# lzzcd001/MeshDiffusion

Hardware: NVIDIA H100
Metric: denoising sample-steps/sec at res-64 (4x64^3), uncond_gen PC sampler (higher is better)
Workload: dtype bf16x3

## Files before the change

### meshdiffusion_b200/csrc/gemm_tc.cuh

```cuda
#pragma once
#include "ptx.cuh"
#include "act_format.cuh"
#include "gn_stats.cuh"

namespace mdb {

constexpr int kBlockM = 128;
constexpr int kRowBytes = 128;
constexpr int kAStageRows = 160;
constexpr int kAStageBytes = kAStageRows * kRowBytes;
constexpr int kMaxLoads = 2048;
constexpr int kMaxAMaps = 16;
constexpr int kGemmThreads = 384;
constexpr int kEpiThreads = 256;

struct __align__(16) LoadEntry {
  uint8_t tmap;
  uint8_t nk;
  uint8_t rows;
  uint8_t jrows;
  int8_t dx, dy, dz;
  uint8_t wsrc;
  uint16_t c0;
  uint16_t wc0;
  uint8_t tap0;
  uint8_t tapj;
  uint8_t tmap_lo;
  uint8_t pad;
};
static_assert(sizeof(LoadEntry) == 16, "LoadEntry must be 16 bytes");

struct GemmSeg {
  int n_groups;
  int nk;
  int a_bytes;
  int a_stride;
  int jbytes;
};
constexpr int kMaxSegs = 8;

struct GemmParams {
  CUtensorMap amap[kMaxAMaps];
  CUtensorMap bmap;
  const LoadEntry* loads;
  int n_loads;
  int n_segs;
  GemmSeg segs[kMaxSegs];
  int bx, by, bz, bb;
  int X, Y, Z, Bn;
  int tx, ty, tz, tb;
  int n_tiles_n;
  int N;
  int b_batched;
  int splits;
  int total_groups;
  float* partial;
  long long split_stride;
  int batch_fastest;
  int kb_elems;
  int b_explicit_k;
  int b_kstep;
  int b_lo_k;
  int n_aslots, a_slot_bytes, n_bslots, b_slot_bytes;
  long long out_lo_off, res_lo_off;
  void* out;
  long long osx, osy, osz, osb;
  long long ocs;
  int out_fp32;
  int round_out;
  const float* bias;
  int bias_on_m;
  const float* rowbias;
  long long rowbias_ld;
  const void* res;
  long long rsx, rsy, rsz, rsb;
  int res_fp32;
  float alpha;
  long long* stats;
  const void* res1;
  long long r1sx, r1sy, r1sz, r1sb;
  long long res1_lo_off;
  int res_c0;
  const float4* gnb_c;
  int gnb_silu;
  int gnb_drop_thresh; float gnb_drop_scale; unsigned long long gnb_seed;
  float* gnb_part;
};

constexpr int kMaxSlots = 8;
constexpr int kMaxDynSmem = 232448;
template <int BLOCK_N, bool kWholeTile = false>
struct GemmCfg {
  static constexpr int kBTileBytes = BLOCK_N * kRowBytes;
  static constexpr int kStatsFloats = 24 * BLOCK_N;
  static constexpr int kStageCols = (kWholeTile || BLOCK_N < 64) ? BLOCK_N : 64;
  static constexpr int kStageRounds = BLOCK_N / kStageCols;
  static_assert(kStageRounds <= 2, "the epilogue stages at most two rounds");
  static constexpr int kAccPitch = kStageCols + 4;
  static constexpr int kAccFloats = kBlockM * kAccPitch;
  static constexpr int kFixedBytes = 1024 + kAccFloats * 4 + kStatsFloats * 4 + 4 * kMaxSlots * 8;
};
constexpr int kRegsProducer = 40, kRegsConsumer = 232;

__device__ __forceinline__ uint64_t kdesc(uint32_t saddr) { return make_wgmma_desc(saddr, 16, 1024); }

template <int OFF>
__device__ __forceinline__ void colsum_butterfly(float (&s)[32], float (&ss)[32], int lane) {
  const bool hi = (lane & OFF) != 0;
#pragma unroll
  for (int i = 0; i < OFF; ++i) {
    const float send_s = hi ? s[i] : s[i + OFF];
    const float send_q = hi ? ss[i] : ss[i + OFF];
    const float keep_s = hi ? s[i + OFF] : s[i];
    const float keep_q = hi ? ss[i + OFF] : ss[i];
    s[i] = keep_s + __shfl_xor_sync(0xffffffffu, send_s, OFF);
    ss[i] = keep_q + __shfl_xor_sync(0xffffffffu, send_q, OFF);
  }
  if constexpr (OFF > 1) colsum_butterfly<OFF / 2>(s, ss, lane);
}

template <int BLOCK_N, bool TF32, bool GNB = false, bool X3 = false>
__global__ void __launch_bounds__(kGemmThreads, 1) gemm_tc_kernel(const __grid_constant__ GemmParams p) {
  using Cfg = GemmCfg<BLOCK_N, GNB>;
  constexpr int kParts = X3 ? 2 : 1;
  const int NA = p.n_aslots, NB = p.n_bslots;
  const uint32_t a_slot = (uint32_t)p.a_slot_bytes, b_slot = (uint32_t)p.b_slot_bytes;
  extern __shared__ uint8_t smem_raw[];
  uint8_t* smem = reinterpret_cast<uint8_t*>((reinterpret_cast<uintptr_t>(smem_raw) + 1023) & ~uintptr_t(1023));
  float* s_acc = reinterpret_cast<float*>(smem + NA * p.a_slot_bytes + NB * p.b_slot_bytes);
  float* s_stats = s_acc + Cfg::kAccFloats;
  uint64_t* bars = reinterpret_cast<uint64_t*>(s_stats + Cfg::kStatsFloats);

  const uint32_t a_ring = smem_u32(smem), b_ring = a_ring + NA * a_slot;
  const uint32_t a_full = smem_u32(bars), a_empty = a_full + 8 * kMaxSlots;
  const uint32_t b_full = a_empty + 8 * kMaxSlots, b_empty = b_full + 8 * kMaxSlots;

  const int warp = __shfl_sync(0xffffffffu, (int)(threadIdx.x >> 5), 0), lane = threadIdx.x & 31;

  if (warp == 0 && lane == 0) {
    for (int i = 0; i < kMaxAMaps; ++i) tma_prefetch_desc(&p.amap[i]);
    tma_prefetch_desc(&p.bmap);
  }
  if (warp == 1 && lane == 0) {
    for (int i = 0; i < NA; ++i) { mbar_init(a_full + 8 * i, 1); mbar_init(a_empty + 8 * i, 2); }
    for (int i = 0; i < NB; ++i) { mbar_init(b_full + 8 * i, 1); mbar_init(b_empty + 8 * i, 2); }
    fence_barrier_init();
    fence_proxy_async();
  }
  __syncthreads();

  const int tiles_m = p.tx * p.ty * p.tz * p.tb;
  const int splits = p.splits > 1 ? p.splits : 1;
  const int total_tiles = tiles_m * p.n_tiles_n * splits;
  const int first_tile = (int)blockIdx.x;
  const int tile_step = (int)gridDim.x;

  auto split_range = [&](int item, int& lo, int& hi) {
    const int sidx = item % splits;
    lo = (int)((long long)p.total_groups * sidx / splits);
    hi = (int)((long long)p.total_groups * (sidx + 1) / splits);
  };
  int mt_of_tile = 0;
  auto decode = [&](int tile, int& x0, int& y0, int& z0, int& b0, int& n0) {
    tile /= splits;
    int nt = tile % p.n_tiles_n;
    int mt = tile / p.n_tiles_n;
    mt_of_tile = mt;
    n0 = nt * BLOCK_N;
    int bt = 0;
    if (p.batch_fastest) { bt = mt % p.tb; mt /= p.tb; }
    int xt = mt % p.tx; mt /= p.tx;
    int yt = mt % p.ty; mt /= p.ty;
    int zt = mt % p.tz; mt /= p.tz;
    if (!p.batch_fastest) bt = mt;
    x0 = xt * p.bx; y0 = yt * p.by; z0 = zt * p.bz; b0 = bt * p.bb;
  };

  if (warp < 4) {
    setmaxnreg_dec<kRegsProducer>();
    if (warp == 0) {
      uint32_t as = 0, aph = 0, bs = 0, bph = 0;
      for (int tile = first_tile; tile < total_tiles; tile += tile_step) {
        int x0, y0, z0, b0, n0;
        decode(tile, x0, y0, z0, b0, n0);
        int kcol = 0, l = 0, gi = 0, g_lo, g_hi;
        split_range(tile, g_lo, g_hi);
        const int bcoord = p.b_batched ? b0 : 0;
        for (int sg = 0; sg < p.n_segs; ++sg) {
          const GemmSeg& seg = p.segs[sg];
          for (int g = 0; g < seg.n_groups; ++g, ++gi) {
            if (gi < g_lo || gi >= g_hi) {
              kcol += seg.nk * p.b_kstep;
              ++l;
              continue;
            }
            const uint4 raw = __ldg(reinterpret_cast<const uint4*>(p.loads + l));
            const LoadEntry& en = reinterpret_cast<const LoadEntry&>(raw);
            mbar_wait(a_empty + 8 * as, aph ^ 1);
            if (elect_one()) {
              const uint32_t abase = a_ring + as * a_slot, bar = a_full + 8 * as;
              mbar_expect_tx(bar, kParts * seg.a_bytes);
              tma_load_5d(&p.amap[en.tmap], bar, abase, en.c0, x0 + en.dx, y0 + en.dy, z0 + en.dz, b0);
              if constexpr (X3) tma_load_5d(&p.amap[en.tmap_lo], bar, abase + seg.a_stride, en.c0, x0 + en.dx, y0 + en.dy, z0 + en.dz, b0);
            }
            __syncwarp();
            if (++as == (uint32_t)NA) { as = 0; aph ^= 1; }
            int kc = (X3 && p.b_explicit_k) ? (int)en.wc0 : kcol;
            for (int j = 0; j < seg.nk; ++j) {
              mbar_wait(b_empty + 8 * bs, bph ^ 1);
              if (elect_one()) {
                const uint32_t bbase = b_ring + bs * b_slot, bar = b_full + 8 * bs;
                mbar_expect_tx(bar, kParts * Cfg::kBTileBytes);
                tma_load_3d(&p.bmap, bar, bbase, kc, n0, bcoord);
                if constexpr (X3) tma_load_3d(&p.bmap, bar, bbase + Cfg::kBTileBytes, kc + p.b_lo_k, n0, bcoord);
              }
              __syncwarp();
              kc += p.b_kstep;
              if (++bs == (uint32_t)NB) { bs = 0; bph ^= 1; }
            }
            kcol += seg.nk * p.b_kstep;
            ++l;
          }
        }
      }
    }
  } else {
    setmaxnreg_inc<kRegsConsumer>();
    const int wg = (warp - 4) >> 2;
    const int wt = threadIdx.x & 127;
    const int q = warp & 3;
    const int half = (warp - 4) >> 2;
    constexpr int kChunks = BLOCK_N / 32;
    constexpr int kChunkStep = kChunks >= 2 ? 2 : 1;
    const int row = q * 32 + lane;
    const int et = threadIdx.x - 128;
    const int rows_per_b = p.bx * p.by * p.bz;
    const int seg = row / rows_per_b;
    int it = 0;
    int staged_n0 = -1, staged_b0 = -1, bias_buf = 0;
    int want_cols = 0;
    if constexpr (GNB) {
      want_cols = (p.stats != nullptr || p.gnb_part != nullptr) ? 1 : 0;
      asm volatile("" : "+r"(want_cols));
    }
    uint32_t as = 0, aph = 0, bs = 0, bph = 0;
    for (int tile = first_tile; tile < total_tiles; tile += tile_step, ++it) {
      const int vit = it;
      constexpr int kAccRegs = X3 ? BLOCK_N : BLOCK_N / 2;
      float acc[kAccRegs];
      float (&acc_hi)[BLOCK_N / 2] = *reinterpret_cast<float (*)[BLOCK_N / 2]>(acc);
#pragma unroll
      for (int i = 0; i < kAccRegs; ++i) acc[i] = 0.f;
      {
        int gi = 0, g_lo, g_hi;
        split_range(tile, g_lo, g_hi);
        int prev_b = -1, prev_a = -1;
        const uint32_t a_row0 = (uint32_t)wg * 64 * kRowBytes;
        for (int sg = 0; sg < p.n_segs; ++sg) {
          const GemmSeg& sgm = p.segs[sg];
          for (int g = 0; g < sgm.n_groups; ++g, ++gi) {
            if (gi < g_lo || gi >= g_hi) continue;
            mbar_wait(a_full + 8 * as, aph);
            const uint32_t abase = a_ring + as * a_slot + a_row0;
            for (int j = 0; j < sgm.nk; ++j) {
              mbar_wait(b_full + 8 * bs, bph);
              const uint64_t ad = kdesc(abase + j * sgm.jbytes);
              const uint64_t bd = kdesc(b_ring + bs * b_slot);
              wgmma_fence();
              if constexpr (X3) {
                const uint64_t adl = kdesc(abase + sgm.a_stride + j * sgm.jbytes);
#pragma unroll
                for (int k = 0; k < kRowBytes / 32; ++k) wgmma_kmajor<2 * BLOCK_N, false>(acc, ad + 2 * k, bd + 2 * k, 1u);
                wgmma_fence();
#pragma unroll
                for (int k = 0; k < kRowBytes / 32; ++k) wgmma_kmajor<BLOCK_N, false>(acc_hi, adl + 2 * k, bd + 2 * k, 1u);
              } else {
#pragma unroll
                for (int k = 0; k < kRowBytes / 32; ++k) wgmma_kmajor<BLOCK_N, TF32>(acc, ad + 2 * k, bd + 2 * k, 1u);
              }
              wgmma_commit();
              wgmma_wait<1>();
              if (wt == 0) {
                if (prev_b >= 0) mbar_arrive(b_empty + 8 * prev_b);
                if (prev_a >= 0) mbar_arrive(a_empty + 8 * prev_a);
              }
              prev_b = (int)bs;
              prev_a = j + 1 == sgm.nk ? (int)as : -1;
              if (++bs == (uint32_t)NB) { bs = 0; bph ^= 1; }
            }
            if (++as == (uint32_t)NA) { as = 0; aph ^= 1; }
          }
        }
        wgmma_wait<0>();
        fence_operands(acc);
        if (wt == 0) {
          if (prev_b >= 0) mbar_arrive(b_empty + 8 * prev_b);
          if (prev_a >= 0) mbar_arrive(a_empty + 8 * prev_a);
        }
        if constexpr (X3) {
#pragma unroll
          for (int i = 0; i < BLOCK_N / 2; ++i) acc[i] += acc[BLOCK_N / 2 + i];
        }
      }
      int x0, y0, z0, b0, n0;
      decode(tile, x0, y0, z0, b0, n0);
      int r = row;
      const int xl = r % p.bx; r /= p.bx;
      const int yl = r % p.by; r /= p.by;
      const int zl = r % p.bz; r /= p.bz;
      const int xg = x0 + xl, yg = y0 + yl, zg = z0 + zl, bg = b0 + r;
      const bool valid = (xg < p.X) && (yg < p.Y) && (zg < p.Z) && (bg < p.Bn);
      const long long ooff = xg * p.osx + yg * p.osy + zg * p.osz + bg * p.osb;
      const long long roff = xg * p.rsx + yg * p.rsy + zg * p.rsz + bg * p.rsb;

      constexpr int kRoundRegs = Cfg::kStageCols / 2;
      auto stage = [&]() {
        const int w4 = (warp & 3), srow = wg * 64 + w4 * 16 + (lane >> 2), scol = 2 * (lane & 3);
#pragma unroll
        for (int j = 0; j < Cfg::kStageCols / 8; ++j) {
          *reinterpret_cast<float2*>(s_acc + srow * Cfg::kAccPitch + 8 * j + scol) = make_float2(acc[4 * j], acc[4 * j + 1]);
          *reinterpret_cast<float2*>(s_acc + (srow + 8) * Cfg::kAccPitch + 8 * j + scol) = make_float2(acc[4 * j + 2], acc[4 * j + 3]);
        }
      };
      named_bar_sync(2, kEpiThreads);
      stage();
      if constexpr (Cfg::kStageRounds > 1) {
#pragma unroll
        for (int i = 0; i < kRoundRegs; ++i) acc[i] = acc[kRoundRegs + i];
      }

      const int bkey = p.rowbias ? b0 : 0;
      if (n0 != staged_n0 || bkey != staged_b0) {
        staged_n0 = n0; staged_b0 = bkey;
        bias_buf ^= 1;
        float* wb = s_stats + 16 * BLOCK_N + bias_buf * 4 * BLOCK_N;
        for (int i = et; i < p.bb * BLOCK_N; i += kEpiThreads) {
          const int sg = i / BLOCK_N, c = i % BLOCK_N;
          const int n = n0 + c, bgl = b0 + sg;
          float bv = 0.f;
          if (n < p.N) {
            if (p.bias && !p.bias_on_m) bv += __ldg(p.bias + n);
            if (p.rowbias && bgl < p.Bn) bv += __ldg(p.rowbias + static_cast<long long>(bgl) * p.rowbias_ld + n);
          }
          wb[i] = bv;
        }
      }
      const float* s_bias = s_stats + 16 * BLOCK_N + bias_buf * 4 * BLOCK_N;
      float* s_part = s_stats + (vit & 1) * 8 * BLOCK_N;
      uint4 rbuf[8];
      auto prefetch_res = [&](int ch) {
        const int nbp = n0 + ch * 32;
        if (!(p.res && valid && p.ocs == 1 && nbp + 32 <= p.N)) return;
        if constexpr (GNB) {
          const bool second = p.res1 && nbp >= p.res_c0;
          const __nv_bfloat16* base = reinterpret_cast<const __nv_bfloat16*>(second ? p.res1 : p.res);
          const long long off = second ? xg * p.r1sx + yg * p.r1sy + zg * p.r1sz + bg * p.r1sb + (nbp - p.res_c0) : roff + nbp;
          const uint4* rp = reinterpret_cast<const uint4*>(base + off);
#pragma unroll
          for (int i = 0; i < 4; ++i) rbuf[i] = __ldg(rp + i);
          if constexpr (X3) {
            const uint4* rl = reinterpret_cast<const uint4*>(base + off + (second ? p.res1_lo_off : p.res_lo_off));
#pragma unroll
            for (int i = 0; i < 4; ++i) rbuf[4 + i] = __ldg(rl + i);
          }
          return;
        }
        if (TF32 || p.res_fp32) {
          const uint4* rp = reinterpret_cast<const uint4*>(reinterpret_cast<const float*>(p.res) + roff + nbp);
#pragma unroll
          for (int i = 0; i < 8; ++i) rbuf[i] = __ldg(rp + i);
        } else {
          const uint4* rp = reinterpret_cast<const uint4*>(reinterpret_cast<const __nv_bfloat16*>(p.res) + roff + nbp);
#pragma unroll
          for (int i = 0; i < 4; ++i) rbuf[i] = __ldg(rp + i);
          if constexpr (X3) {
            const uint4* rl = reinterpret_cast<const uint4*>(reinterpret_cast<const __nv_bfloat16*>(p.res) + roff + nbp + p.res_lo_off);
#pragma unroll
            for (int i = 0; i < 4; ++i) rbuf[4 + i] = __ldg(rl + i);
          }
        }
      };
      const int ch0 = kChunkStep == 2 ? half : 0;
      const bool active = kChunkStep == 2 || half == 0;
      if (active) prefetch_res(ch0);

      constexpr int kRoundChunks = Cfg::kStageCols / 32;
#pragma unroll 1
      for (int rnd = 0; rnd < Cfg::kStageRounds; ++rnd) {
        if (rnd > 0) {
          named_bar_sync(2, kEpiThreads);
          stage();
        }
        named_bar_sync(2, kEpiThreads);

#pragma unroll 1
        for (int ch = ch0 + rnd * kRoundChunks; ch < (rnd + 1) * kRoundChunks && active; ch += kChunkStep) {
          uint32_t rr[32];
          {
            const float4* src = reinterpret_cast<const float4*>(s_acc + row * Cfg::kAccPitch + (ch - rnd * kRoundChunks) * 32);
#pragma unroll
            for (int i = 0; i < 8; ++i) {
              const float4 t = src[i];
              rr[4 * i] = __float_as_uint(t.x); rr[4 * i + 1] = __float_as_uint(t.y);
              rr[4 * i + 2] = __float_as_uint(t.z); rr[4 * i + 3] = __float_as_uint(t.w);
            }
          }
          const int nb = n0 + ch * 32;
          if (nb >= p.N) continue;
          if (splits > 1) {
            if (valid) {
              float* pp = p.partial + (long long)(tile % splits) * p.split_stride + (X3 ? (ooff >> 1) : ooff) + nb;
              if (nb + 32 <= p.N) {
#pragma unroll
                for (int i = 0; i < 8; ++i)
                  reinterpret_cast<float4*>(pp)[i] = make_float4(__uint_as_float(rr[4 * i]), __uint_as_float(rr[4 * i + 1]),
                                                                 __uint_as_float(rr[4 * i + 2]), __uint_as_float(rr[4 * i + 3]));
              } else {
                for (int i = 0; i < 32; ++i) if (nb + i < p.N) pp[i] = __uint_as_float(rr[i]);
              }
            }
            continue;
          }
          const bool full = (nb + 32 <= p.N) && (p.ocs == 1);
          float v[32];
          const float mbias = (p.bias && p.bias_on_m && valid) ? __ldg(p.bias + xg) : 0.f;
          const float* sb = s_bias + (seg < 4 ? seg : 0) * BLOCK_N + ch * 32;
#pragma unroll
          for (int i = 0; i < 32; ++i) v[i] = __uint_as_float(rr[i]) * p.alpha + mbias + sb[i];
          float q2[GNB ? 32 : 1];
          if constexpr (GNB) {
            if (valid) {
              const float4* cc = p.gnb_c + static_cast<long long>(bg) * p.N + nb;
              unsigned long long hsh[8];
              if (p.gnb_drop_thresh > 0) {
                const unsigned long long e4 = (unsigned long long)((((static_cast<long long>(bg) * p.Z + zg) * p.Y + yg) * p.X + xg) * p.N + nb) >> 2;
#pragma unroll
                for (int i = 0; i < 8; ++i) hsh[i] = drop_hash64(p.gnb_seed, e4 + i);
              }
#pragma unroll
              for (int i = 0; i < 32; ++i) {
                const float4 kc = __ldg(cc + i);
                const __nv_bfloat16 xb = reinterpret_cast<const __nv_bfloat16*>(rbuf)[i];
                float xv = __bfloat162float(xb);
                if constexpr (X3) xv += __bfloat162float(reinterpret_cast<const __nv_bfloat16*>(rbuf + 4)[i]);
                float d = v[i];
                if (p.gnb_drop_thresh > 0) {
                  const unsigned r16 = (unsigned)((hsh[i >> 2] >> (16 * (i & 3))) & 0xFFFFu);
                  d = r16 >= (unsigned)p.gnb_drop_thresh ? d * p.gnb_drop_scale : 0.f;
                }
                if (p.gnb_silu) {
                  const float h = fmaf(xv, kc.x, kc.y);
                  d *= X3 ? dsilu_ex2_half(h) : dsilu_tanh_half(h);
                }
                v[i] = d;
                q2[i] = d * fmaf(xv, kc.z, kc.w);
              }
            } else {
#pragma unroll
              for (int i = 0; i < 32; ++i) q2[i] = 0.f;
            }
          }
          if (!GNB && p.res && valid) {
            if (TF32 || p.res_fp32) {
              if (full) {
#pragma unroll
                for (int i = 0; i < 8; ++i) {
                  const float4 t = *reinterpret_cast<const float4*>(&rbuf[i]);
                  v[4 * i] += t.x; v[4 * i + 1] += t.y; v[4 * i + 2] += t.z; v[4 * i + 3] += t.w;
                }
              } else {
                const float* rp = reinterpret_cast<const float*>(p.res) + roff + nb;
                for (int i = 0; i < 32; ++i) if (nb + i < p.N) v[i] += rp[i];
              }
            } else {
              if (full) {
#pragma unroll
                for (int i = 0; i < 4; ++i) {
                  const __nv_bfloat162* h = reinterpret_cast<const __nv_bfloat162*>(&rbuf[i]);
#pragma unroll
                  for (int j = 0; j < 4; ++j) {
                    float2 f = __bfloat1622float2(h[j]);
                    if constexpr (X3) {
                      const float2 l = __bfloat1622float2(reinterpret_cast<const __nv_bfloat162*>(&rbuf[4 + i])[j]);
                      f.x += l.x; f.y += l.y;
                    }
                    v[8 * i + 2 * j] += f.x; v[8 * i + 2 * j + 1] += f.y;
                  }
                }
              } else {
                const __nv_bfloat16* rp = reinterpret_cast<const __nv_bfloat16*>(p.res) + roff + nb;
                for (int i = 0; i < 32; ++i)
                  if (nb + i < p.N) v[i] += __bfloat162float(rp[i]) + (X3 ? __bfloat162float(rp[i + p.res_lo_off]) : 0.f);
              }
            }
          }
          if (ch + kChunkStep < kChunks) prefetch_res(ch + kChunkStep);
          if (valid) {
            if (TF32 || p.out_fp32) {
              float* op = reinterpret_cast<float*>(p.out) + ooff + nb;
              if (full) {
#pragma unroll
                for (int i = 0; i < 8; ++i) {
                  float4 t = make_float4(v[4 * i], v[4 * i + 1], v[4 * i + 2], v[4 * i + 3]);
                  if (p.round_out) { t.x = to_tf32_rna(t.x); t.y = to_tf32_rna(t.y); t.z = to_tf32_rna(t.z); t.w = to_tf32_rna(t.w); }
                  reinterpret_cast<float4*>(op)[i] = t;
                }
              } else {
                for (int i = 0; i < 32; ++i) if (nb + i < p.N) op[i * p.ocs] = v[i];
              }
            } else {
              __nv_bfloat16* op = reinterpret_cast<__nv_bfloat16*>(p.out) + ooff + nb;
              if (full) {
#pragma unroll
                for (int i = 0; i < 4; ++i) {
                  uint4 t;
                  __nv_bfloat162* h = reinterpret_cast<__nv_bfloat162*>(&t);
#pragma unroll
                  for (int j = 0; j < 4; ++j) h[j] = __floats2bfloat162_rn(v[8 * i + 2 * j], v[8 * i + 2 * j + 1]);
                  reinterpret_cast<uint4*>(op)[i] = t;
                  if constexpr (X3) {
                    uint4 tl;
                    __nv_bfloat162* l = reinterpret_cast<__nv_bfloat162*>(&tl);
#pragma unroll
                    for (int j = 0; j < 4; ++j) {
                      const float2 f = __bfloat1622float2(h[j]);
                      l[j] = __floats2bfloat162_rn(v[8 * i + 2 * j] - f.x, v[8 * i + 2 * j + 1] - f.y);
                    }
                    reinterpret_cast<uint4*>(op + p.out_lo_off)[i] = tl;
                  }
                }
              } else {
                for (int i = 0; i < 32; ++i)
                  if (nb + i < p.N) {
                    const __nv_bfloat16 hb = __float2bfloat16(v[i]);
                    op[i * p.ocs] = hb;
                    if constexpr (X3) op[i * p.ocs + p.out_lo_off] = __float2bfloat16(v[i] - __bfloat162float(hb));
                  }
              }
            }
          }
          if (GNB ? (want_cols != 0) : (p.stats != nullptr)) {
            float s[32], ss[32];
#pragma unroll
            for (int i = 0; i < 32; ++i) {
              const float t = valid ? v[i] : 0.f;
              s[i] = t; ss[i] = GNB ? q2[GNB ? i : 0] : t * t;
            }
            colsum_butterfly<16>(s, ss, lane);
            s_part[(q * 2 + 0) * BLOCK_N + ch * 32 + lane] = s[0];
            s_part[(q * 2 + 1) * BLOCK_N + ch * 32 + lane] = ss[0];
          }
        }
      }
      if constexpr (GNB) {
        if (p.gnb_part && splits == 1) {
          named_bar_sync(1, kEpiThreads);
          const int warps_per_seg = rows_per_b >= 128 ? 4 : rows_per_b / 32;
          for (int i = et; i < p.bb * BLOCK_N; i += kEpiThreads) {
            const int sg = i / BLOCK_N, c = i % BLOCK_N;
            const int n = n0 + c;
            if (mt_of_tile < tiles_m && n < p.N) {
              float ts = 0.f, tq = 0.f;
              for (int w = sg * warps_per_seg; w < (sg + 1) * warps_per_seg; ++w) {
                ts += s_part[(w * 2 + 0) * BLOCK_N + c];
                tq += s_part[(w * 2 + 1) * BLOCK_N + c];
              }
              float* dst = p.gnb_part + ((static_cast<long long>(mt_of_tile) * p.bb + sg) * p.N + n) * 2;
              dst[0] = ts; dst[1] = tq;
            }
          }
        }
      }
      if (!GNB && p.stats && splits == 1) {
        named_bar_sync(1, kEpiThreads);
        const int warps_per_seg = rows_per_b >= 128 ? 4 : rows_per_b / 32;
        for (int i0 = 0; i0 < p.bb * BLOCK_N; i0 += kEpiThreads) {
          const int i = i0 + et;
          const int sg = i / BLOCK_N, c = i % BLOCK_N;
          const int bgl = b0 + sg, n = n0 + c;
          if (i < p.bb * BLOCK_N && bgl < p.Bn && n < p.N) {
            float ts = 0.f, tq = 0.f;
            for (int w = sg * warps_per_seg; w < (sg + 1) * warps_per_seg; ++w) {
              ts += s_part[(w * 2 + 0) * BLOCK_N + c];
              tq += s_part[(w * 2 + 1) * BLOCK_N + c];
            }
            long long* dst = p.stats + (static_cast<long long>(bgl) * p.N + n) * kStatWords;
            stat_add(dst, ts);
            stat_add(dst + 2, tq);
          }
        }
      }
    }
  }
}

}
```

### meshdiffusion_b200/csrc/ptx.cuh

```cuda
#pragma once
#include <cuda.h>
#include <cuda_runtime.h>
#include <cuda_bf16.h>
#include <stdint.h>
#include <stdio.h>

namespace mdb {

__device__ __forceinline__ uint32_t smem_u32(const void* p) {
  return static_cast<uint32_t>(__cvta_generic_to_shared(p));
}

__device__ __forceinline__ void mbar_init(uint32_t bar, uint32_t count) {
  asm volatile("mbarrier.init.shared::cta.b64 [%0], %1;" ::"r"(bar), "r"(count) : "memory");
}
__device__ __forceinline__ void fence_barrier_init() {
  asm volatile("fence.mbarrier_init.release.cluster;" ::: "memory");
}
__device__ __forceinline__ void fence_proxy_async() {
  asm volatile("fence.proxy.async.shared::cta;" ::: "memory");
}
__device__ __forceinline__ void mbar_expect_tx(uint32_t bar, uint32_t bytes) {
  asm volatile("mbarrier.arrive.expect_tx.shared::cta.b64 _, [%0], %1;" ::"r"(bar), "r"(bytes) : "memory");
}
__device__ __forceinline__ void mbar_arrive(uint32_t bar) {
  asm volatile("mbarrier.arrive.shared::cta.b64 _, [%0];" ::"r"(bar) : "memory");
}
__device__ __forceinline__ void mbar_wait(uint32_t bar, uint32_t parity) {
  asm volatile(
      "{\n\t.reg .pred p;\n\t.reg .u32 n;\n\tmov.u32 n, 0;\n"
      "MDB_WAIT:\n\t"
      "mbarrier.try_wait.parity.shared::cta.b64 p, [%0], %1;\n\t"
      "@p bra MDB_DONE;\n\t"
      "add.u32 n, n, 1;\n\t"
      "setp.lt.u32 p, n, 16777216;\n\t"
      "@p bra MDB_WAIT;\n\t"
      "trap;\n"
      "MDB_DONE:\n\t}"
      :: "r"(bar), "r"(parity) : "memory");
}

__device__ __forceinline__ void tma_prefetch_desc(const void* desc) {
  asm volatile("prefetch.tensormap [%0];" ::"l"(reinterpret_cast<uint64_t>(desc)) : "memory");
}
__device__ __forceinline__ void tma_load_5d(const void* desc, uint32_t bar, uint32_t dst, int c0, int c1, int c2,
                                            int c3, int c4) {
  asm volatile(
      "cp.async.bulk.tensor.5d.shared::cluster.global.mbarrier::complete_tx::bytes"
      " [%0], [%1, {%3, %4, %5, %6, %7}], [%2];"
      :
      : "r"(dst), "l"(reinterpret_cast<uint64_t>(desc)), "r"(bar), "r"(c0), "r"(c1), "r"(c2), "r"(c3), "r"(c4)
      : "memory");
}
__device__ __forceinline__ void tma_load_3d(const void* desc, uint32_t bar, uint32_t dst, int c0, int c1, int c2) {
  asm volatile(
      "cp.async.bulk.tensor.3d.shared::cluster.global.mbarrier::complete_tx::bytes"
      " [%0], [%1, {%3, %4, %5}], [%2];"
      :
      : "r"(dst), "l"(reinterpret_cast<uint64_t>(desc)), "r"(bar), "r"(c0), "r"(c1), "r"(c2)
      : "memory");
}

__device__ __forceinline__ uint64_t make_wgmma_desc(uint32_t saddr, uint32_t lbo_bytes, uint32_t sbo_bytes) {
  return static_cast<uint64_t>((saddr & 0x3FFFFu) >> 4) | (static_cast<uint64_t>((lbo_bytes >> 4) & 0x3FFFu) << 16) |
         (static_cast<uint64_t>((sbo_bytes >> 4) & 0x3FFFu) << 32) | (static_cast<uint64_t>(1) << 62);
}
__device__ __forceinline__ void wgmma_fence() { asm volatile("wgmma.fence.sync.aligned;" ::: "memory"); }
__device__ __forceinline__ void wgmma_commit() { asm volatile("wgmma.commit_group.sync.aligned;" ::: "memory"); }
template <int N>
__device__ __forceinline__ void wgmma_wait() { asm volatile("wgmma.wait_group.sync.aligned %0;" ::"n"(N) : "memory"); }
template <int N>
__device__ __forceinline__ void fence_operands(float (&d)[N]) {
#pragma unroll
  for (int i = 0; i < N; ++i) asm volatile("" : "+f"(d[i])::"memory");
}

template <int TA, int TB>
__device__ __forceinline__ void wgmma_m64n32k16_bf16(float (&d)[16], uint64_t a, uint64_t b, uint32_t scale_d) {
  asm volatile(
      "{\n\t.reg .pred p;\n\tsetp.ne.b32 p, %18, 0;\n\t"
      "wgmma.mma_async.sync.aligned.m64n32k16.f32.bf16.bf16 "
      "{%0, %1, %2, %3, %4, %5, %6, %7, %8, %9, %10, %11, %12, %13, %14, %15}, "
      "%16, %17, p, 1, 1, %19, %20;\n\t}"
      : "+f"(d[0]), "+f"(d[1]), "+f"(d[2]), "+f"(d[3]), "+f"(d[4]), "+f"(d[5]), "+f"(d[6]), "+f"(d[7]), "+f"(d[8]), "+f"(d[9]), "+f"(d[10]), "+f"(d[11]), "+f"(d[12]), "+f"(d[13]), "+f"(d[14]), "+f"(d[15])
      : "l"(a), "l"(b), "r"(scale_d), "n"(TA), "n"(TB));
}
__device__ __forceinline__ void wgmma_m64n32k8_tf32(float (&d)[16], uint64_t a, uint64_t b, uint32_t scale_d) {
  asm volatile(
      "{\n\t.reg .pred p;\n\tsetp.ne.b32 p, %18, 0;\n\t"
      "wgmma.mma_async.sync.aligned.m64n32k8.f32.tf32.tf32 "
      "{%0, %1, %2, %3, %4, %5, %6, %7, %8, %9, %10, %11, %12, %13, %14, %15}, "
      "%16, %17, p, 1, 1;\n\t}"
      : "+f"(d[0]), "+f"(d[1]), "+f"(d[2]), "+f"(d[3]), "+f"(d[4]), "+f"(d[5]), "+f"(d[6]), "+f"(d[7]), "+f"(d[8]), "+f"(d[9]), "+f"(d[10]), "+f"(d[11]), "+f"(d[12]), "+f"(d[13]), "+f"(d[14]), "+f"(d[15])
      : "l"(a), "l"(b), "r"(scale_d));
}
template <int TA, int TB>
__device__ __forceinline__ void wgmma_m64n128k16_bf16(float (&d)[64], uint64_t a, uint64_t b, uint32_t scale_d) {
  asm volatile(
      "{\n\t.reg .pred p;\n\tsetp.ne.b32 p, %66, 0;\n\t"
      "wgmma.mma_async.sync.aligned.m64n128k16.f32.bf16.bf16 "
      "{%0, %1, %2, %3, %4, %5, %6, %7, %8, %9, %10, %11, %12, %13, %14, %15, %16, %17, %18, %19, %20, %21, %22, %23, %24, %25, %26, %27, %28, %29, %30, %31, %32, %33, %34, %35, %36, %37, %38, %39, %40, %41, %42, %43, %44, %45, %46, %47, %48, %49, %50, %51, %52, %53, %54, %55, %56, %57, %58, %59, %60, %61, %62, %63}, "
      "%64, %65, p, 1, 1, %67, %68;\n\t}"
      : "+f"(d[0]), "+f"(d[1]), "+f"(d[2]), "+f"(d[3]), "+f"(d[4]), "+f"(d[5]), "+f"(d[6]), "+f"(d[7]), "+f"(d[8]), "+f"(d[9]), "+f"(d[10]), "+f"(d[11]), "+f"(d[12]), "+f"(d[13]), "+f"(d[14]), "+f"(d[15]), "+f"(d[16]), "+f"(d[17]), "+f"(d[18]), "+f"(d[19]), "+f"(d[20]), "+f"(d[21]), "+f"(d[22]), "+f"(d[23]), "+f"(d[24]), "+f"(d[25]), "+f"(d[26]), "+f"(d[27]), "+f"(d[28]), "+f"(d[29]), "+f"(d[30]), "+f"(d[31]), "+f"(d[32]), "+f"(d[33]), "+f"(d[34]), "+f"(d[35]), "+f"(d[36]), "+f"(d[37]), "+f"(d[38]), "+f"(d[39]), "+f"(d[40]), "+f"(d[41]), "+f"(d[42]), "+f"(d[43]), "+f"(d[44]), "+f"(d[45]), "+f"(d[46]), "+f"(d[47]), "+f"(d[48]), "+f"(d[49]), "+f"(d[50]), "+f"(d[51]), "+f"(d[52]), "+f"(d[53]), "+f"(d[54]), "+f"(d[55]), "+f"(d[56]), "+f"(d[57]), "+f"(d[58]), "+f"(d[59]), "+f"(d[60]), "+f"(d[61]), "+f"(d[62]), "+f"(d[63])
      : "l"(a), "l"(b), "r"(scale_d), "n"(TA), "n"(TB));
}
__device__ __forceinline__ void wgmma_m64n128k8_tf32(float (&d)[64], uint64_t a, uint64_t b, uint32_t scale_d) {
  asm volatile(
      "{\n\t.reg .pred p;\n\tsetp.ne.b32 p, %66, 0;\n\t"
      "wgmma.mma_async.sync.aligned.m64n128k8.f32.tf32.tf32 "
      "{%0, %1, %2, %3, %4, %5, %6, %7, %8, %9, %10, %11, %12, %13, %14, %15, %16, %17, %18, %19, %20, %21, %22, %23, %24, %25, %26, %27, %28, %29, %30, %31, %32, %33, %34, %35, %36, %37, %38, %39, %40, %41, %42, %43, %44, %45, %46, %47, %48, %49, %50, %51, %52, %53, %54, %55, %56, %57, %58, %59, %60, %61, %62, %63}, "
      "%64, %65, p, 1, 1;\n\t}"
      : "+f"(d[0]), "+f"(d[1]), "+f"(d[2]), "+f"(d[3]), "+f"(d[4]), "+f"(d[5]), "+f"(d[6]), "+f"(d[7]), "+f"(d[8]), "+f"(d[9]), "+f"(d[10]), "+f"(d[11]), "+f"(d[12]), "+f"(d[13]), "+f"(d[14]), "+f"(d[15]), "+f"(d[16]), "+f"(d[17]), "+f"(d[18]), "+f"(d[19]), "+f"(d[20]), "+f"(d[21]), "+f"(d[22]), "+f"(d[23]), "+f"(d[24]), "+f"(d[25]), "+f"(d[26]), "+f"(d[27]), "+f"(d[28]), "+f"(d[29]), "+f"(d[30]), "+f"(d[31]), "+f"(d[32]), "+f"(d[33]), "+f"(d[34]), "+f"(d[35]), "+f"(d[36]), "+f"(d[37]), "+f"(d[38]), "+f"(d[39]), "+f"(d[40]), "+f"(d[41]), "+f"(d[42]), "+f"(d[43]), "+f"(d[44]), "+f"(d[45]), "+f"(d[46]), "+f"(d[47]), "+f"(d[48]), "+f"(d[49]), "+f"(d[50]), "+f"(d[51]), "+f"(d[52]), "+f"(d[53]), "+f"(d[54]), "+f"(d[55]), "+f"(d[56]), "+f"(d[57]), "+f"(d[58]), "+f"(d[59]), "+f"(d[60]), "+f"(d[61]), "+f"(d[62]), "+f"(d[63])
      : "l"(a), "l"(b), "r"(scale_d));
}

template <int TA, int TB>
__device__ __forceinline__ void wgmma_m64n64k16_bf16(float (&d)[32], uint64_t a, uint64_t b, uint32_t scale_d) {
  asm volatile(
      "{\n\t.reg .pred p;\n\tsetp.ne.b32 p, %34, 0;\n\t"
      "wgmma.mma_async.sync.aligned.m64n64k16.f32.bf16.bf16 "
      "{%0, %1, %2, %3, %4, %5, %6, %7, %8, %9, %10, %11, %12, %13, %14, %15, %16, %17, %18, %19, %20, %21, %22, %23, %24, %25, %26, %27, %28, %29, %30, %31}, "
      "%32, %33, p, 1, 1, %35, %36;\n\t}"
      : "+f"(d[0]), "+f"(d[1]), "+f"(d[2]), "+f"(d[3]), "+f"(d[4]), "+f"(d[5]), "+f"(d[6]), "+f"(d[7]), "+f"(d[8]), "+f"(d[9]), "+f"(d[10]), "+f"(d[11]), "+f"(d[12]), "+f"(d[13]), "+f"(d[14]), "+f"(d[15]), "+f"(d[16]), "+f"(d[17]), "+f"(d[18]), "+f"(d[19]), "+f"(d[20]), "+f"(d[21]), "+f"(d[22]), "+f"(d[23]), "+f"(d[24]), "+f"(d[25]), "+f"(d[26]), "+f"(d[27]), "+f"(d[28]), "+f"(d[29]), "+f"(d[30]), "+f"(d[31])
      : "l"(a), "l"(b), "r"(scale_d), "n"(TA), "n"(TB));
}
template <int TA, int TB>
__device__ __forceinline__ void wgmma_m64n256k16_bf16(float (&d)[128], uint64_t a, uint64_t b, uint32_t scale_d) {
  asm volatile(
      "{\n\t.reg .pred p;\n\tsetp.ne.b32 p, %130, 0;\n\t"
      "wgmma.mma_async.sync.aligned.m64n256k16.f32.bf16.bf16 "
      "{%0, %1, %2, %3, %4, %5, %6, %7, %8, %9, %10, %11, %12, %13, %14, %15, %16, %17, %18, %19, %20, %21, %22, %23, %24, %25, %26, %27, %28, %29, %30, %31, %32, %33, %34, %35, %36, %37, %38, %39, %40, %41, %42, %43, %44, %45, %46, %47, %48, %49, %50, %51, %52, %53, %54, %55, %56, %57, %58, %59, %60, %61, %62, %63, %64, %65, %66, %67, %68, %69, %70, %71, %72, %73, %74, %75, %76, %77, %78, %79, %80, %81, %82, %83, %84, %85, %86, %87, %88, %89, %90, %91, %92, %93, %94, %95, %96, %97, %98, %99, %100, %101, %102, %103, %104, %105, %106, %107, %108, %109, %110, %111, %112, %113, %114, %115, %116, %117, %118, %119, %120, %121, %122, %123, %124, %125, %126, %127}, "
      "%128, %129, p, 1, 1, %131, %132;\n\t}"
      : "+f"(d[0]), "+f"(d[1]), "+f"(d[2]), "+f"(d[3]), "+f"(d[4]), "+f"(d[5]), "+f"(d[6]), "+f"(d[7]), "+f"(d[8]), "+f"(d[9]), "+f"(d[10]), "+f"(d[11]), "+f"(d[12]), "+f"(d[13]), "+f"(d[14]), "+f"(d[15]), "+f"(d[16]), "+f"(d[17]), "+f"(d[18]), "+f"(d[19]), "+f"(d[20]), "+f"(d[21]), "+f"(d[22]), "+f"(d[23]), "+f"(d[24]), "+f"(d[25]), "+f"(d[26]), "+f"(d[27]), "+f"(d[28]), "+f"(d[29]), "+f"(d[30]), "+f"(d[31]), "+f"(d[32]), "+f"(d[33]), "+f"(d[34]), "+f"(d[35]), "+f"(d[36]), "+f"(d[37]), "+f"(d[38]), "+f"(d[39]), "+f"(d[40]), "+f"(d[41]), "+f"(d[42]), "+f"(d[43]), "+f"(d[44]), "+f"(d[45]), "+f"(d[46]), "+f"(d[47]), "+f"(d[48]), "+f"(d[49]), "+f"(d[50]), "+f"(d[51]), "+f"(d[52]), "+f"(d[53]), "+f"(d[54]), "+f"(d[55]), "+f"(d[56]), "+f"(d[57]), "+f"(d[58]), "+f"(d[59]), "+f"(d[60]), "+f"(d[61]), "+f"(d[62]), "+f"(d[63]), "+f"(d[64]), "+f"(d[65]), "+f"(d[66]), "+f"(d[67]), "+f"(d[68]), "+f"(d[69]), "+f"(d[70]), "+f"(d[71]), "+f"(d[72]), "+f"(d[73]), "+f"(d[74]), "+f"(d[75]), "+f"(d[76]), "+f"(d[77]), "+f"(d[78]), "+f"(d[79]), "+f"(d[80]), "+f"(d[81]), "+f"(d[82]), "+f"(d[83]), "+f"(d[84]), "+f"(d[85]), "+f"(d[86]), "+f"(d[87]), "+f"(d[88]), "+f"(d[89]), "+f"(d[90]), "+f"(d[91]), "+f"(d[92]), "+f"(d[93]), "+f"(d[94]), "+f"(d[95]), "+f"(d[96]), "+f"(d[97]), "+f"(d[98]), "+f"(d[99]), "+f"(d[100]), "+f"(d[101]), "+f"(d[102]), "+f"(d[103]), "+f"(d[104]), "+f"(d[105]), "+f"(d[106]), "+f"(d[107]), "+f"(d[108]), "+f"(d[109]), "+f"(d[110]), "+f"(d[111]), "+f"(d[112]), "+f"(d[113]), "+f"(d[114]), "+f"(d[115]), "+f"(d[116]), "+f"(d[117]), "+f"(d[118]), "+f"(d[119]), "+f"(d[120]), "+f"(d[121]), "+f"(d[122]), "+f"(d[123]), "+f"(d[124]), "+f"(d[125]), "+f"(d[126]), "+f"(d[127])
      : "l"(a), "l"(b), "r"(scale_d), "n"(TA), "n"(TB));
}

template <int N, bool TF32>
__device__ __forceinline__ void wgmma_kmajor(float (&d)[N / 2], uint64_t a, uint64_t b, uint32_t scale_d) {
  if constexpr (N == 256) {
    static_assert(!TF32, "m64n256 is used by the split-bf16 products only");
    wgmma_m64n256k16_bf16<0, 0>(d, a, b, scale_d);
  } else if constexpr (N == 128) {
    if constexpr (TF32) wgmma_m64n128k8_tf32(d, a, b, scale_d); else wgmma_m64n128k16_bf16<0, 0>(d, a, b, scale_d);
  } else if constexpr (N == 64) {
    static_assert(!TF32, "m64n64 is used by the split-bf16 products only");
    wgmma_m64n64k16_bf16<0, 0>(d, a, b, scale_d);
  } else {
    static_assert(N == 32, "wgmma_kmajor is instantiated for N = 32, 64, 128 and 256");
    if constexpr (TF32) wgmma_m64n32k8_tf32(d, a, b, scale_d); else wgmma_m64n32k16_bf16<0, 0>(d, a, b, scale_d);
  }
}

__device__ __forceinline__ bool elect_one() {
  uint32_t pred = 0;
  asm volatile(
      "{\n\t.reg .pred p;\n\t"
      "elect.sync _|p, 0xffffffff;\n\t"
      "selp.u32 %0, 1, 0, p;\n\t}"
      : "=r"(pred));
  return pred != 0;
}

template <int N>
__device__ __forceinline__ void setmaxnreg_inc() { asm volatile("setmaxnreg.inc.sync.aligned.u32 %0;" ::"n"(N)); }
template <int N>
__device__ __forceinline__ void setmaxnreg_dec() { asm volatile("setmaxnreg.dec.sync.aligned.u32 %0;" ::"n"(N)); }

__device__ __forceinline__ void named_bar_sync(int id, int nthreads) {
  asm volatile("bar.sync %0, %1;" ::"r"(id), "r"(nthreads) : "memory");
}

}
```

Before: 36.02.

## Ping-pong consumer warpgroups across tiles and use register-A wgmma for split-bf16

For non-GNB GEMMs, each consumer warpgroup now owns whole 128-row tiles, alternating between the two groups. New mbarriers pass the MMA turn and the staging buffer between them, so one group's epilogue overlaps the other's mainloop. Each consumer skips the ring slots used by its partner's tile and keeps two 64-row accumulator halves. The X3 (bf16x3) path at BLOCK_N=128 loads the A-hi fragment once via ldmatrix into registers and issues three wgmmas (hi*hi, hi*lo, lo*hi) per k-step instead of a merged double-width accumulator. This raises register pressure and synchronisation complexity, and risks serialising MMAs if the turn handoff stalls.

```diff
diff --git a/meshdiffusion_b200/csrc/gemm_tc.cuh b/meshdiffusion_b200/csrc/gemm_tc.cuh
--- a/meshdiffusion_b200/csrc/gemm_tc.cuh
+++ b/meshdiffusion_b200/csrc/gemm_tc.cuh
@@ -98,7 +98,7 @@
   static_assert(kStageRounds <= 2, "the epilogue stages at most two rounds");
   static constexpr int kAccPitch = kStageCols + 4;
   static constexpr int kAccFloats = kBlockM * kAccPitch;
-  static constexpr int kFixedBytes = 1024 + kAccFloats * 4 + kStatsFloats * 4 + 4 * kMaxSlots * 8;
+  static constexpr int kFixedBytes = 1024 + kAccFloats * 4 + kStatsFloats * 4 + (4 * kMaxSlots + 4) * 8;
 };
 constexpr int kRegsProducer = 40, kRegsConsumer = 232;
 
@@ -122,6 +122,7 @@
 template <int BLOCK_N, bool TF32, bool GNB = false, bool X3 = false>
 __global__ void __launch_bounds__(kGemmThreads, 1) gemm_tc_kernel(const __grid_constant__ GemmParams p) {
   using Cfg = GemmCfg<BLOCK_N, GNB>;
+  constexpr bool kPP = !GNB;
   constexpr int kParts = X3 ? 2 : 1;
   const int NA = p.n_aslots, NB = p.n_bslots;
   const uint32_t a_slot = (uint32_t)p.a_slot_bytes, b_slot = (uint32_t)p.b_slot_bytes;
@@ -134,6 +135,7 @@
   const uint32_t a_ring = smem_u32(smem), b_ring = a_ring + NA * a_slot;
   const uint32_t a_full = smem_u32(bars), a_empty = a_full + 8 * kMaxSlots;
   const uint32_t b_full = a_empty + 8 * kMaxSlots, b_empty = b_full + 8 * kMaxSlots;
+  const uint32_t mma_turn = b_empty + 8 * kMaxSlots, stage_free = mma_turn + 16;
 
   const int warp = __shfl_sync(0xffffffffu, (int)(threadIdx.x >> 5), 0), lane = threadIdx.x & 31;
 
@@ -142,8 +144,10 @@
     tma_prefetch_desc(&p.bmap);
   }
   if (warp == 1 && lane == 0) {
-    for (int i = 0; i < NA; ++i) { mbar_init(a_full + 8 * i, 1); mbar_init(a_empty + 8 * i, 2); }
-    for (int i = 0; i < NB; ++i) { mbar_init(b_full + 8 * i, 1); mbar_init(b_empty + 8 * i, 2); }
+    constexpr uint32_t kReaders = kPP ? 1 : 2;
+    for (int i = 0; i < NA; ++i) { mbar_init(a_full + 8 * i, 1); mbar_init(a_empty + 8 * i, kReaders); }
+    for (int i = 0; i < NB; ++i) { mbar_init(b_full + 8 * i, 1); mbar_init(b_empty + 8 * i, kReaders); }
+    for (int i = 0; i < 2; ++i) { mbar_init(mma_turn + 8 * i, 1); mbar_init(stage_free + 8 * i, 1); }
     fence_barrier_init();
     fence_proxy_async();
   }
@@ -229,56 +233,114 @@
     const int wg = (warp - 4) >> 2;
     const int wt = threadIdx.x & 127;
     const int q = warp & 3;
-    const int half = (warp - 4) >> 2;
+    const int half = kPP ? 0 : wg;
     constexpr int kChunks = BLOCK_N / 32;
-    constexpr int kChunkStep = kChunks >= 2 ? 2 : 1;
+    constexpr int kChunkStep = (!kPP && kChunks >= 2) ? 2 : 1;
+    constexpr int kEpi = kPP ? 128 : kEpiThreads;
+    const int ebar = kPP ? 1 + wg : 2;
     const int row = q * 32 + lane;
-    const int et = threadIdx.x - 128;
+    const int et = kPP ? wt : threadIdx.x - 128;
     const int rows_per_b = p.bx * p.by * p.bz;
     const int seg = row / rows_per_b;
     int it = 0;
-    int staged_n0 = -1, staged_b0 = -1, bias_buf = 0;
+    int staged_n0 = -1, staged_b0 = -1, bias_buf = kPP ? wg : 0;
     int want_cols = 0;
     if constexpr (GNB) {
       want_cols = (p.stats != nullptr || p.gnb_part != nullptr) ? 1 : 0;
       asm volatile("" : "+r"(want_cols));
     }
     uint32_t as = 0, aph = 0, bs = 0, bph = 0;
-    for (int tile = first_tile; tile < total_tiles; tile += tile_step, ++it) {
+    uint32_t turn_ph = 0, free_ph = 0;
+    auto skip_item = [&](int item) {
+      int g_lo, g_hi, g0 = 0, na = 0, nb = 0;
+      split_range(item, g_lo, g_hi);
+      for (int sg = 0; sg < p.n_segs; ++sg) {
+        const int lo = max(g_lo, g0), hi = min(g_hi, g0 + p.segs[sg].n_groups);
+        if (hi > lo) { na += hi - lo; nb += (hi - lo) * p.segs[sg].nk; }
+        g0 += p.segs[sg].n_groups;
+      }
+      as += na; aph ^= (as / NA) & 1; as %= NA;
+      bs += nb; bph ^= (bs / NB) & 1; bs %= NB;
+    };
+    for (int tile = first_tile + (kPP ? wg * tile_step : 0); tile < total_tiles; tile += (kPP ? 2 : 1) * tile_step, ++it) {
       const int vit = it;
-      constexpr int kAccRegs = X3 ? BLOCK_N : BLOCK_N / 2;
-      float acc[kAccRegs];
-      float (&acc_hi)[BLOCK_N / 2] = *reinterpret_cast<float (*)[BLOCK_N / 2]>(acc);
-#pragma unroll
-      for (int i = 0; i < kAccRegs; ++i) acc[i] = 0.f;
+      if constexpr (kPP) {
+        if (tile != first_tile) {
+          skip_item(tile - tile_step);
+          mbar_wait(mma_turn + 8 * wg, turn_ph);
+          turn_ph ^= 1;
+        }
+      }
+      constexpr int kHalves = kPP ? 2 : 1;
+      constexpr bool kMerged = X3 && !(kPP && BLOCK_N == 128);
+      constexpr int kAccRegs = kMerged ? BLOCK_N : BLOCK_N / 2;
+      float acc[kHalves][kAccRegs];
+#pragma unroll
+      for (int h = 0; h < kHalves; ++h)
+#pragma unroll
+        for (int i = 0; i < kAccRegs; ++i) acc[h][i] = 0.f;
       {
         int gi = 0, g_lo, g_hi;
         split_range(tile, g_lo, g_hi);
         int prev_b = -1, prev_a = -1;
-        const uint32_t a_row0 = (uint32_t)wg * 64 * kRowBytes;
         for (int sg = 0; sg < p.n_segs; ++sg) {
           const GemmSeg& sgm = p.segs[sg];
           for (int g = 0; g < sgm.n_groups; ++g, ++gi) {
             if (gi < g_lo || gi >= g_hi) continue;
             mbar_wait(a_full + 8 * as, aph);
-            const uint32_t abase = a_ring + as * a_slot + a_row0;
+            const uint32_t abase = a_ring + as * a_slot;
             for (int j = 0; j < sgm.nk; ++j) {
               mbar_wait(b_full + 8 * bs, bph);
-              const uint64_t ad = kdesc(abase + j * sgm.jbytes);
-              const uint64_t bd = kdesc(b_ring + bs * b_slot);
-              wgmma_fence();
-              if constexpr (X3) {
-                const uint64_t adl = kdesc(abase + sgm.a_stride + j * sgm.jbytes);
-#pragma unroll
-                for (int k = 0; k < kRowBytes / 32; ++k) wgmma_kmajor<2 * BLOCK_N, false>(acc, ad + 2 * k, bd + 2 * k, 1u);
+              const uint32_t bbase = b_ring + bs * b_slot;
+              const uint64_t bd = kdesc(bbase);
+              if constexpr (X3 && !kMerged) {
+                static_assert(BLOCK_N == 128, "the register-A split-bf16 form is built for BLOCK_N = 128");
+                const int mi = lane >> 3, rr = lane & 7;
+                const uint32_t lrow = (uint32_t)(16 * (warp & 3) + 8 * (mi & 1) + rr) * kRowBytes;
+                const uint64_t bdl = kdesc(bbase + Cfg::kBTileBytes);
+#pragma unroll
+                for (int h = 0; h < kHalves; ++h) {
+                  const uint32_t arow = abase + (uint32_t)h * 64 * kRowBytes + j * sgm.jbytes;
+                  uint32_t ahi[kRowBytes / 32][4];
+#pragma unroll
+                  for (int k = 0; k < kRowBytes / 32; ++k)
+                    ldmatrix_x4(ahi[k], arow + lrow + ((uint32_t)((2 * k + (mi >> 1)) ^ rr) << 4));
+                  const uint64_t adl = kdesc(arow + sgm.a_stride);
+                  wgmma_fence();
+#pragma unroll
+                  for (int k = 0; k < kRowBytes / 32; ++k) {
+                    wgmma_m64n128k16_bf16_rs<0>(acc[h], ahi[k], bd + 2 * k, 1u);
+                    wgmma_m64n128k16_bf16_rs<0>(acc[h], ahi[k], bdl + 2 * k, 1u);
+                    wgmma_kmajor<BLOCK_N, false>(acc[h], adl + 2 * k, bd + 2 * k, 1u);
+                  }
+                  wgmma_commit();
+                  if (h == 0) wgmma_wait<1>();
+                }
+              } else {
                 wgmma_fence();
 #pragma unroll
-                for (int k = 0; k < kRowBytes / 32; ++k) wgmma_kmajor<BLOCK_N, false>(acc_hi, adl + 2 * k, bd + 2 * k, 1u);
-              } else {
-#pragma unroll
-                for (int k = 0; k < kRowBytes / 32; ++k) wgmma_kmajor<BLOCK_N, TF32>(acc, ad + 2 * k, bd + 2 * k, 1u);
-              }
-              wgmma_commit();
+                for (int h = 0; h < kHalves; ++h) {
+                  const uint64_t ad = kdesc(abase + (uint32_t)(kPP ? h : wg) * 64 * kRowBytes + j * sgm.jbytes);
+                  if constexpr (kMerged) {
+#pragma unroll
+                    for (int k = 0; k < kRowBytes / 32; ++k) wgmma_kmajor<2 * BLOCK_N, false>(acc[h], ad + 2 * k, bd + 2 * k, 1u);
+                  } else {
+#pragma unroll
+                    for (int k = 0; k < kRowBytes / 32; ++k) wgmma_kmajor<BLOCK_N, TF32>(acc[h], ad + 2 * k, bd + 2 * k, 1u);
+                  }
+                }
+              }
+              if constexpr (kMerged) {
+                wgmma_fence();
+#pragma unroll
+                for (int h = 0; h < kHalves; ++h) {
+                  float (&acc_hi)[BLOCK_N / 2] = *reinterpret_cast<float (*)[BLOCK_N / 2]>(acc[h]);
+                  const uint64_t adl = kdesc(abase + (uint32_t)(kPP ? h : wg) * 64 * kRowBytes + sgm.a_stride + j * sgm.jbytes);
+#pragma unroll
+                  for (int k = 0; k < kRowBytes / 32; ++k) wgmma_kmajor<BLOCK_N, false>(acc_hi, adl + 2 * k, bd + 2 * k, 1u);
+                }
+              }
+              if constexpr (!(X3 && !kMerged)) wgmma_commit();
               wgmma_wait<1>();
               if (wt == 0) {
                 if (prev_b >= 0) mbar_arrive(b_empty + 8 * prev_b);
@@ -291,15 +353,21 @@
             if (++as == (uint32_t)NA) { as = 0; aph ^= 1; }
           }
         }
+        if constexpr (kPP) {
+          if (wt == 0) mbar_arrive(mma_turn + 8 * (wg ^ 1));
+        }
         wgmma_wait<0>();
-        fence_operands(acc);
+#pragma unroll
+        for (int h = 0; h < kHalves; ++h) fence_operands(acc[h]);
         if (wt == 0) {
           if (prev_b >= 0) mbar_arrive(b_empty + 8 * prev_b);
           if (prev_a >= 0) mbar_arrive(a_empty + 8 * prev_a);
         }
-        if constexpr (X3) {
-#pragma unroll
-          for (int i = 0; i < BLOCK_N / 2; ++i) acc[i] += acc[BLOCK_N / 2 + i];
+        if constexpr (kMerged) {
+#pragma unroll
+          for (int h = 0; h < kHalves; ++h)
+#pragma unroll
+            for (int i = 0; i < BLOCK_N / 2; ++i) acc[h][i] += acc[h][BLOCK_N / 2 + i];
         }
       }
       int x0, y0, z0, b0, n0;
@@ -315,26 +383,38 @@
 
       constexpr int kRoundRegs = Cfg::kStageCols / 2;
       auto stage = [&]() {
-        const int w4 = (warp & 3), srow = wg * 64 + w4 * 16 + (lane >> 2), scol = 2 * (lane & 3);
-#pragma unroll
-        for (int j = 0; j < Cfg::kStageCols / 8; ++j) {
-          *reinterpret_cast<float2*>(s_acc + srow * Cfg::kAccPitch + 8 * j + scol) = make_float2(acc[4 * j], acc[4 * j + 1]);
-          *reinterpret_cast<float2*>(s_acc + (srow + 8) * Cfg::kAccPitch + 8 * j + scol) = make_float2(acc[4 * j + 2], acc[4 * j + 3]);
+#pragma unroll
+        for (int h = 0; h < kHalves; ++h) {
+          const int w4 = (warp & 3), srow = (kPP ? h : wg) * 64 + w4 * 16 + (lane >> 2), scol = 2 * (lane & 3);
+#pragma unroll
+          for (int j = 0; j < Cfg::kStageCols / 8; ++j) {
+            *reinterpret_cast<float2*>(s_acc + srow * Cfg::kAccPitch + 8 * j + scol) = make_float2(acc[h][4 * j], acc[h][4 * j + 1]);
+            *reinterpret_cast<float2*>(s_acc + (srow + 8) * Cfg::kAccPitch + 8 * j + scol) = make_float2(acc[h][4 * j + 2], acc[h][4 * j + 3]);
+          }
         }
       };
-      named_bar_sync(2, kEpiThreads);
+      if constexpr (kPP) {
+        if (tile != first_tile) {
+          mbar_wait(stage_free + 8 * wg, free_ph);
+          free_ph ^= 1;
+        }
+      } else {
+        named_bar_sync(ebar, kEpi);
+      }
       stage();
       if constexpr (Cfg::kStageRounds > 1) {
 #pragma unroll
-        for (int i = 0; i < kRoundRegs; ++i) acc[i] = acc[kRoundRegs + i];
+        for (int h = 0; h < kHalves; ++h)
+#pragma unroll
+          for (int i = 0; i < kRoundRegs; ++i) acc[h][i] = acc[h][kRoundRegs + i];
       }
 
       const int bkey = p.rowbias ? b0 : 0;
       if (n0 != staged_n0 || bkey != staged_b0) {
         staged_n0 = n0; staged_b0 = bkey;
-        bias_buf ^= 1;
+        if constexpr (!kPP) bias_buf ^= 1;
         float* wb = s_stats + 16 * BLOCK_N + bias_buf * 4 * BLOCK_N;
-        for (int i = et; i < p.bb * BLOCK_N; i += kEpiThreads) {
+        for (int i = et; i < p.bb * BLOCK_N; i += kEpi) {
           const int sg = i / BLOCK_N, c = i % BLOCK_N;
           const int n = n0 + c, bgl = b0 + sg;
           float bv = 0.f;
@@ -346,7 +426,7 @@
         }
       }
       const float* s_bias = s_stats + 16 * BLOCK_N + bias_buf * 4 * BLOCK_N;
-      float* s_part = s_stats + (vit & 1) * 8 * BLOCK_N;
+      float* s_part = s_stats + (kPP ? wg : (vit & 1)) * 8 * BLOCK_N;
       uint4 rbuf[8];
       auto prefetch_res = [&](int ch) {
         const int nbp = n0 + ch * 32;
@@ -388,10 +468,10 @@
 #pragma unroll 1
       for (int rnd = 0; rnd < Cfg::kStageRounds; ++rnd) {
         if (rnd > 0) {
-          named_bar_sync(2, kEpiThreads);
+          named_bar_sync(ebar, kEpi);
           stage();
         }
-        named_bar_sync(2, kEpiThreads);
+        named_bar_sync(ebar, kEpi);
 
 #pragma unroll 1
         for (int ch = ch0 + rnd * kRoundChunks; ch < (rnd + 1) * kRoundChunks && active; ch += kChunkStep) {
@@ -571,10 +651,13 @@
           }
         }
       }
+      if constexpr (kPP) {
+        named_bar_sync(ebar, kEpi);
+        if (wt == 0) mbar_arrive(stage_free + 8 * (wg ^ 1));
+      }
       if (!GNB && p.stats && splits == 1) {
-        named_bar_sync(1, kEpiThreads);
         const int warps_per_seg = rows_per_b >= 128 ? 4 : rows_per_b / 32;
-        for (int i0 = 0; i0 < p.bb * BLOCK_N; i0 += kEpiThreads) {
+        for (int i0 = 0; i0 < p.bb * BLOCK_N; i0 += kEpi) {
           const int i = i0 + et;
           const int sg = i / BLOCK_N, c = i % BLOCK_N;
           const int bgl = b0 + sg, n = n0 + c;
diff --git a/meshdiffusion_b200/csrc/ptx.cuh b/meshdiffusion_b200/csrc/ptx.cuh
--- a/meshdiffusion_b200/csrc/ptx.cuh
+++ b/meshdiffusion_b200/csrc/ptx.cuh
@@ -114,6 +114,21 @@
       : "l"(a), "l"(b), "r"(scale_d));
 }
 
+template <int TB>
+__device__ __forceinline__ void wgmma_m64n128k16_bf16_rs(float (&d)[64], const uint32_t (&a)[4], uint64_t b, uint32_t scale_d) {
+  asm volatile(
+      "{\n\t.reg .pred p;\n\tsetp.ne.b32 p, %69, 0;\n\t"
+      "wgmma.mma_async.sync.aligned.m64n128k16.f32.bf16.bf16 "
+      "{%0, %1, %2, %3, %4, %5, %6, %7, %8, %9, %10, %11, %12, %13, %14, %15, %16, %17, %18, %19, %20, %21, %22, %23, %24, %25, %26, %27, %28, %29, %30, %31, %32, %33, %34, %35, %36, %37, %38, %39, %40, %41, %42, %43, %44, %45, %46, %47, %48, %49, %50, %51, %52, %53, %54, %55, %56, %57, %58, %59, %60, %61, %62, %63}, "
+      "{%64, %65, %66, %67}, %68, p, 1, 1, %70;\n\t}"
+      : "+f"(d[0]), "+f"(d[1]), "+f"(d[2]), "+f"(d[3]), "+f"(d[4]), "+f"(d[5]), "+f"(d[6]), "+f"(d[7]), "+f"(d[8]), "+f"(d[9]), "+f"(d[10]), "+f"(d[11]), "+f"(d[12]), "+f"(d[13]), "+f"(d[14]), "+f"(d[15]), "+f"(d[16]), "+f"(d[17]), "+f"(d[18]), "+f"(d[19]), "+f"(d[20]), "+f"(d[21]), "+f"(d[22]), "+f"(d[23]), "+f"(d[24]), "+f"(d[25]), "+f"(d[26]), "+f"(d[27]), "+f"(d[28]), "+f"(d[29]), "+f"(d[30]), "+f"(d[31]), "+f"(d[32]), "+f"(d[33]), "+f"(d[34]), "+f"(d[35]), "+f"(d[36]), "+f"(d[37]), "+f"(d[38]), "+f"(d[39]), "+f"(d[40]), "+f"(d[41]), "+f"(d[42]), "+f"(d[43]), "+f"(d[44]), "+f"(d[45]), "+f"(d[46]), "+f"(d[47]), "+f"(d[48]), "+f"(d[49]), "+f"(d[50]), "+f"(d[51]), "+f"(d[52]), "+f"(d[53]), "+f"(d[54]), "+f"(d[55]), "+f"(d[56]), "+f"(d[57]), "+f"(d[58]), "+f"(d[59]), "+f"(d[60]), "+f"(d[61]), "+f"(d[62]), "+f"(d[63])
+      : "r"(a[0]), "r"(a[1]), "r"(a[2]), "r"(a[3]), "l"(b), "r"(scale_d), "n"(TB));
+}
+__device__ __forceinline__ void ldmatrix_x4(uint32_t (&r)[4], uint32_t saddr) {
+  asm volatile("ldmatrix.sync.aligned.m8n8.x4.shared.b16 {%0, %1, %2, %3}, [%4];"
+               : "=r"(r[0]), "=r"(r[1]), "=r"(r[2]), "=r"(r[3]) : "r"(saddr) : "memory");
+}
+
 template <int TA, int TB>
 __device__ __forceinline__ void wgmma_m64n64k16_bf16(float (&d)[32], uint64_t a, uint64_t b, uint32_t scale_d) {
   asm volatile(
```

New measurement: 36.55 (median of 6 runs). 1.5% higher.
